# sikoba/babble

Hardware: AMD Instinct MI355X
Metric: ECDSA event verifies/sec (higher is better)
Workload: dtype u32; 1 GPU; C2: VerifyBatch of 1M signed Events per GPU (64 creators, 1x64-B tx, ~446-B bodies); per-key tables rebuilt every step; events_per_gpu=1000000, creators=64, parallelism=single, batches_in_flight=2

## Files before the change

### babble_amd/csrc/kernels.hip

```cpp
#include <hip/hip_runtime.h>
#include <stdint.h>

#include <algorithm>
#include <cstdlib>

#include "evjson.h"
#include "hostscalar.h"

#include "verify_core.h"


#ifndef BV_SHA_WAVES
#define BV_SHA_WAVES 1
#endif
__global__ void __launch_bounds__(256, BV_SHA_WAVES) k_sha256(uint64_t n_msgs, const uint8_t *__restrict__ bytes,
                                                const uint64_t *__restrict__ off,
                                                uint32_t *__restrict__ digest_words, uint64_t max_len) {
  const uint64_t m = (uint64_t)blockIdx.x * blockDim.x + threadIdx.x;
  if (m < n_msgs && off[m + 1] - off[m] <= max_len) sha256_one(m, bytes, off, digest_words);
}

__global__ void __launch_bounds__(256) k_put_digests(uint64_t n, const uint64_t *__restrict__ idx,
                                                     const uint32_t *__restrict__ vals, uint32_t *__restrict__ dig) {
  const uint64_t t = (uint64_t)blockIdx.x * blockDim.x + threadIdx.x;
// ... 391 lines not shown
__global__ void __launch_bounds__(256) k_table_pair_g(const uint32_t *__restrict__ sub, uint32_t *__restrict__ table,
                                                      uint4 *__restrict__ pscr, uint32_t j, uint32_t c0) {
  constexpr uint32_t E = 16, NS = 1u << L, ENT = 1u << (W - 1);
  const uint32_t c = c0 + blockIdx.x, t = threadIdx.x;
  const uint32_t *s_lo = sub + (uint64_t)(2 * j) * NS * BV_ENTRY_U32;
  const uint32_t *s_hi = s_lo + (uint64_t)NS * BV_ENTRY_U32;
  __shared__ fe sT[511];
  uint4 *ps = pscr + (uint64_t)blockIdx.x * E * 2 * 256 + t;
  fe acc;
  fe_set(acc, 1);
#pragma unroll 1
  for (uint32_t e = 0; e < E; e++) {
    const uint32_t d = k12_digit(4096u * c + 256u * e + t, ENT), lo = d & (NS - 1), hi = d >> L;
    fe x1, y1, x2, y2, H;
    pair_load(s_lo, s_hi, lo, hi, x1, y1, x2, y2);
    pair_denominator(H, pair_kind(lo, hi), x1, x2);
    ps[(2 * e) * 256] = make_uint4(acc.v[0], acc.v[1], acc.v[2], acc.v[3]);
    ps[(2 * e + 1) * 256] = make_uint4(acc.v[4], acc.v[5], acc.v[6], acc.v[7]);
    fe_mul(acc, acc, H);
  }
  fe q = acc;
  block_inverse<256>(sT, q, t);
  uint32_t *base = table + (uint64_t)j * ENT * BV_ENTRY_U32;
#pragma unroll 1
  for (int e = (int)E - 1; e >= 0; e--) {
    const uint32_t d = k12_digit(4096u * c + 256u * e + t, ENT), lo = d & (NS - 1), hi = d >> L;
    const int kind = pair_kind(lo, hi);
    fe x1, y1, x2, y2, H, Hinv, pre;
    pair_load(s_lo, s_hi, lo, hi, x1, y1, x2, y2);
    pair_denominator(H, kind, x1, x2);
    const uint4 p0 = ps[(2 * e) * 256], p1 = ps[(2 * e + 1) * 256];
    pre.v[0] = p0.x; pre.v[1] = p0.y; pre.v[2] = p0.z; pre.v[3] = p0.w;
    pre.v[4] = p1.x; pre.v[5] = p1.y; pre.v[6] = p1.z; pre.v[7] = p1.w;
    fe_mul(Hinv, q, pre);
    fe_mul(q, q, H);
    pair_store(base + (uint64_t)d * BV_ENTRY_U32, nullptr, kind, x1, y1, x2, y2, Hinv);
  }
}

__global__ void __launch_bounds__(256) k_sinv(uint64_t n_items, uint32_t M, const uint32_t *__restrict__ s_be,
                                              const uint8_t *__restrict__ pre, uint32_t *__restrict__ w_out) {
  const uint64_t T = (uint64_t)gridDim.x * blockDim.x;
  const uint64_t t = (uint64_t)blockIdx.x * blockDim.x + threadIdx.x;
  sinv_thread(t, T, n_items, M, s_be, pre, w_out);
}

__device__ __forceinline__ void write_status(uint64_t i, uint64_t hi, uint8_t st, uint8_t *status, uint64_t *bits) {
  if (i < hi) status[i] = st;
  const uint64_t mask = __ballot(i < hi && st == BV_ACCEPT);
  if ((threadIdx.x & 63) == 0 && i < hi) bits[i >> 6] = mask;
}

#ifndef BV_GWAVES
#define BV_GWAVES 1
#endif
#ifndef BV_LWAVES
#define BV_LWAVES 1
#endif
__global__ void __launch_bounds__(256) k_glv_split(uint64_t n_items, const uint32_t *__restrict__ r_be,
                                                   const uint32_t *__restrict__ w_in, uint32_t *__restrict__ u12) {
  const uint64_t i = (uint64_t)blockIdx.x * blockDim.x + threadIdx.x;
  if (i < n_items) glv_split_item(i, r_be, w_in, u12);
}

template <bool LAT, bool SPLIT>
__global__ void __launch_bounds__(256, LAT ? BV_LWAVES : BV_GWAVES) k_verify_g(uint64_t n_items, uint64_t lo, uint64_t hi,
                                                  const uint32_t *__restrict__ item_key,
                                                  const uint32_t *__restrict__ r_be, const uint32_t *__restrict__ s_be,
                                                  const uint8_t *__restrict__ pre, const uint8_t *__restrict__ kstatus,
                                                  const uint32_t *__restrict__ item_msg,
                                                  const uint32_t *__restrict__ digest_words,
                                                  const uint32_t *__restrict__ w_in, uint32_t *__restrict__ u12,
                                                  const uint32_t *__restrict__ g_table, uint32_t *__restrict__ rg) {
  const uint64_t i = lo + (uint64_t)blockIdx.x * blockDim.x + threadIdx.x;
  if (i < hi)
    verify_item_g<LAT, SPLIT>(i, n_items, item_key, r_be, s_be, pre, kstatus, item_msg, digest_words, w_in, u12,
                              g_table, rg);
}

#ifndef BV_QWAVES
#define BV_QWAVES 4
#endif
template <int W, int NWIN, bool LAT>
__global__ void __launch_bounds__(256, LAT ? BV_LWAVES : BV_QWAVES) k_verify_q(uint64_t n_items, uint64_t lo, uint64_t hi,
                                                  const uint32_t *__restrict__ item_key,
                                                  const uint32_t *__restrict__ r_be, const uint32_t *__restrict__ s_be,
                                                  const uint8_t *__restrict__ pre, const uint8_t *__restrict__ kstatus,
                                                  const uint32_t *__restrict__ u12,
                                                  const uint32_t *__restrict__ key_table,
                                                  const uint64_t *__restrict__ key_tabs,
                                                  const uint32_t *__restrict__ rg, uint8_t *__restrict__ status,
                                                  uint64_t *__restrict__ bits) {
  const uint64_t i = lo + (uint64_t)blockIdx.x * blockDim.x + threadIdx.x;
  uint8_t st = BV_REJECT;
  if (i < hi)
    st = verify_item_q<W, NWIN, LAT>(i, n_items, item_key, r_be, s_be, pre, kstatus, u12, key_table, key_tabs, rg);
  write_status(i, hi, st, status, bits);
}

template <int W, int NWIN, bool LAT>
__global__ void __launch_bounds__(256, LAT ? BV_LWAVES : BV_QWAVES) k_verify_qf(uint64_t n_items, uint64_t lo, uint64_t hi,
                                                   const uint32_t *__restrict__ item_key,
                                                   const uint32_t *__restrict__ r_be, const uint32_t *__restrict__ s_be,
                                                   const uint8_t *__restrict__ pre, const uint8_t *__restrict__ kstatus,
                                                   const uint32_t *__restrict__ w_in,
                                                   const uint32_t *__restrict__ key_table,
                                                   const uint64_t *__restrict__ key_tabs, uint32_t *__restrict__ rq) {
// ... 960 lines not shown
```

### babble_amd/csrc/point.h

```cpp
#pragma once
#include "field.h"

struct gej {
  fe X, Y, Z;
};

DEV void gej_double(gej &r, const gej &a) {
  fe A, B, C, D, E, F, t;
  fe_sqr(A, a.X);
  fe_sqr(B, a.Y);
  fe_sqr(C, B);
  fe_add(t, a.X, B);
  fe_sqr(t, t);
  fe_sub(t, t, A);
  fe_sub(t, t, C);
  fe_dbl(D, t);
  fe_dbl(E, A);
  fe_add(E, E, A);
  fe_sqr(F, E);
  fe Z3;
  fe_mul(Z3, a.Y, a.Z);
  fe_dbl(r.Z, Z3);
  fe_dbl(t, D);
  fe_sub(r.X, F, t);
// ... 149 lines not shown
  }
  fe_dbl(I, H);
  fe_sqr(I, I);
  fe_mul(J, H, I);
  fe_dbl(rr, rr);
  fe_mul(V, U1, I);
  fe_add(t, r.Z, b.Z);
  fe_sqr(t, t);
  fe_sub(t, t, Z1Z1);
  fe_sub(t, t, Z2Z2);
  fe_mul(r.Z, t, H);
  fe_sqr(t, rr);
  fe_sub(t, t, J);
  fe_sub(t, t, V);
  fe_sub(r.X, t, V);
  fe_sub(t, V, r.X);
  fe_mul(t, rr, t);
  fe_mul(J, S1, J);
  fe_dbl(J, J);
  fe_sub(r.Y, t, J);
}

struct gexz {
  fe X, Y, ZZ, ZZZ;
};

DEV void gexz_double(gexz &r, const gexz &a) {
  fe U, V, W, S, M, t;
  fe_dbl(U, a.Y);
  fe_sqr(V, U);
  fe_mul(W, U, V);
  fe_mul(S, a.X, V);
  fe_sqr(M, a.X);
  fe_dbl(t, M);
  fe_add(M, M, t);
  fe_sqr(t, M);
  fe_dbl(r.X, S);
  fe_sub(r.X, t, r.X);
  fe_sub(t, S, r.X);
  fe_mul(t, M, t);
  fe_mul(U, W, a.Y);
  fe_sub(r.Y, t, U);
  fe_mul(r.ZZ, V, a.ZZ);
  fe_mul(r.ZZZ, W, a.ZZZ);
}

DEV void gexz_set_ge(gexz &r, const fe &x, const fe &y) {
  r.X = x;
  r.Y = y;
  fe_set(r.ZZ, 1);
  fe_set(r.ZZZ, 1);
}

DEV void gexz_add_ge(gexz &r, bool &inf, const fe &x2, const fe &y2, bool xz_only = false) {
  if (inf) {
    gexz_set_ge(r, x2, y2);
    inf = false;
    return;
  }
  fe P, R, PP, PPP, Q, t;
  fe_mul(P, x2, r.ZZ);
  fe_sub(P, P, r.X);
  fe_mul(R, y2, r.ZZZ);
  fe_sub(R, R, r.Y);
  if (fe_is_zero(P)) {
    if (fe_is_zero(R)) {
      gexz d;
      gexz_double(d, r);
      r = d;
    } else {
      inf = true;
    }
    return;
  }
  fe_sqr(PP, P);
  fe_mul(PPP, P, PP);
  fe_mul(Q, r.X, PP);
  fe_mul(r.ZZ, r.ZZ, PP);
  fe_sqr(t, R);
  fe_sub(t, t, PPP);
  fe_sub(t, t, Q);
  fe_sub(r.X, t, Q);
  if (xz_only) return;
  fe_sub(t, Q, r.X);
  fe_mul(t, R, t);
  fe_mul(r.ZZZ, r.ZZZ, PPP);
  fe_mul(PPP, r.Y, PPP);
  fe_sub(r.Y, t, PPP);
}

DEV void gexz_add_ge_lat(gexz &r, bool &inf, const fe &x2, const fe &y2) {
#if defined(__HIP_DEVICE_COMPILE__)
  if (inf) {
    gexz_set_ge(r, x2, y2);
    inf = false;
    return;
  }
  fe P, R, PP, RR, PPP, Q, ZZ3, t, u;
  fe_mul_mul_zip_asm(P, x2, r.ZZ, R, y2, r.ZZZ);
  fe_sub(P, P, r.X);
  fe_sub(R, R, r.Y);
  if (fe_is_zero(P)) {
    if (fe_is_zero(R)) {
      gexz d;
      gexz_double(d, r);
      r = d;
    } else {
      inf = true;
    }
    return;
  }
  fe_sqr_sqr_zip_asm(PP, P, RR, R);
  fe_mul_mul_mul_zip_asm(PPP, P, PP, Q, r.X, PP, ZZ3, r.ZZ, PP);
  r.ZZ = ZZ3;
  fe_sub(t, RR, PPP);
  fe_sub(t, t, Q);
  fe_sub(r.X, t, Q);
  fe_sub(t, Q, r.X);
  fe_mul_mul_mul_zip_asm(t, R, t, u, r.Y, PPP, ZZ3, r.ZZZ, PPP);
  r.ZZZ = ZZ3;
  fe_sub(r.Y, t, u);
#else
  gexz_add_ge(r, inf, x2, y2);
#endif
}

DEV void gexz_add(gexz &r, bool &rinf, const gexz &b, bool binf) {
  if (binf) return;
  if (rinf) {
    r = b;
    rinf = false;
    return;
  }
  fe U1, U2, S1, S2, P, R, PP, PPP, Q, t;
  fe_mul(U1, r.X, b.ZZ);
  fe_mul(U2, b.X, r.ZZ);
  fe_mul(S1, r.Y, b.ZZZ);
  fe_mul(S2, b.Y, r.ZZZ);
  fe_sub(P, U2, U1);
  fe_sub(R, S2, S1);
  if (fe_is_zero(P)) {
// ... 54 lines not shown
  fe_sub(t, Q, r.X);
  fe_mul_mul_mul_zip_asm(t, R, t, u, S1, PPP, r.ZZZ, W12, PPP);
  fe_sub(r.Y, t, u);
#else
  gexz_add(r, rinf, b, binf);
#endif
}

DEV void gexz_sum_ge_lat(gexz &r, bool &rinf, const fe &x1, const fe &y1, bool i1, const fe &x2, const fe &y2,
                         bool i2) {
  rinf = i1 && i2;
  if (i1 || i2) {
    if (!rinf) gexz_set_ge(r, i1 ? x2 : x1, i1 ? y2 : y1);
    return;
  }
  fe P, R;
  fe_sub(P, x2, x1);
  fe_sub(R, y2, y1);
  if (fe_is_zero(P)) {
    if (fe_is_zero(R)) {
      gexz a;
      gexz_set_ge(a, x1, y1);
      gexz_double(r, a);
    } else {
      rinf = true;
    }
    return;
  }
#if defined(__HIP_DEVICE_COMPILE__)
  fe PP, RR, PPP, Q, t, u;
  fe_sqr_sqr_zip_asm(PP, P, RR, R);
  fe_mul_mul_zip_asm(PPP, P, PP, Q, x1, PP);
  fe_sub(t, RR, PPP);
  fe_sub(t, t, Q);
  fe_sub(r.X, t, Q);
  fe_sub(t, Q, r.X);
  fe_mul_mul_zip_asm(t, R, t, u, y1, PPP);
  fe_sub(r.Y, t, u);
  r.ZZ = PP;
  r.ZZZ = PPP;
#else
  gexz_set_ge(r, x1, y1);
  gexz_add_ge(r, rinf, x2, y2);
#endif
}

DEV void gexz_from_gej(gexz &r, const gej &a) {
  r.X = a.X;
  r.Y = a.Y;
  fe_sqr(r.ZZ, a.Z);
  fe_mul(r.ZZZ, r.ZZ, a.Z);
}

template <bool LAT>
DEV void pt_add_ge(gexz &r, bool &inf, const fe &x2, const fe &y2, bool xz_only = false) {
  if (LAT) gexz_add_ge_lat(r, inf, x2, y2);
  else gexz_add_ge(r, inf, x2, y2, xz_only);
}

template <bool LAT>
DEV void gexz_add_ge_aff(gexz &r, bool &inf, const fe &x2, const fe &y2) {
  fe P, R, PP, RR, PPP, Q, t, u, v;
  fe_sub(P, x2, r.X);
  fe_sub(R, y2, r.Y);
  if (fe_is_zero(P)) {
    if (fe_is_zero(R)) {
      gexz d;
      gexz_double(d, r);
      r = d;
    } else {
      inf = true;
    }
    return;
  }
#if defined(__HIP_DEVICE_COMPILE__)
  if (LAT) {
    fe_sqr_sqr_zip_asm(PP, P, RR, R);
    fe_mul_mul_zip_asm(PPP, P, PP, Q, r.X, PP);
  } else
#endif
  {
    fe_sqr(PP, P);
    fe_sqr(RR, R);
    fe_mul(PPP, P, PP);
    fe_mul(Q, r.X, PP);
  }
  fe_sub(t, RR, PPP);
  fe_sub(t, t, Q);
  fe_sub(t, t, Q);
  fe_sub(u, Q, t);
  r.X = t;
  r.ZZ = PP;
  r.ZZZ = PPP;
#if defined(__HIP_DEVICE_COMPILE__)
  if (LAT) {
    fe_mul_mul_zip_asm(t, R, u, v, r.Y, PPP);
  } else
#endif
  {
    fe_mul(t, R, u);
    fe_mul(v, r.Y, PPP);
  }
  fe_sub(r.Y, t, v);
}

template <bool LAT>
DEV void pt_add_ge_step(gexz &r, bool &inf, const fe &x2, const fe &y2, bool take, bool xz_only = false) {
  if (take) pt_add_ge<LAT>(r, inf, x2, y2, xz_only);
}
template <bool LAT>
DEV void pt_add_ge_step(gej &r, bool &inf, const fe &x2, const fe &y2, bool take, bool xz_only = false) {
  if (take) gej_add_ge_sel<LAT>(r, inf, x2, y2);
}
template <bool LAT>
DEV void pt_add_ge(gej &r, bool &inf, const fe &x2, const fe &y2) {
  gej_add_ge_sel<LAT>(r, inf, x2, y2);
}
```

### babble_amd/csrc/verify_core.h

```cpp
#pragma once
#include <type_traits>
#include <stdint.h>

#include "../../include/babbleverify.h"
#include "geometry.h"
#include "coop.h"
#include "point.h"
#include "sha256.h"

#define KS_OK 0
#define KS_EMPTY 1
#define KS_BAD 2

static constexpr uint32_t P_MINUS_N[8] = {0x2FC9BAEEu, 0x402DA172u, 0x50B75FC4u, 0x45512319u,
                                          0x00000001u, 0u, 0u, 0u};

DEV void fe_load_be(fe &r, const uint8_t *b) {
#pragma unroll
  for (int i = 0; i < 8; i++) {
    const uint8_t *q = b + 4 * (7 - i);
    r.v[i] = ((uint32_t)q[0] << 24) | ((uint32_t)q[1] << 16) | ((uint32_t)q[2] << 8) | q[3];
  }
}
DEV void fe_load_be_words(fe &r, const uint32_t *w) {
// ... 505 lines not shown
};

struct lane_park {
#if defined(__HIP_DEVICE_COMPILE__)
  DEV uint4 *slot() {
    __shared__ uint4 park[BV_STAGE_LANES];
    return park + threadIdx.x;
  }
  DEV void put(const uint32_t v[4]) { *slot() = make_uint4(v[0], v[1], v[2], v[3]); }
  DEV void get(uint32_t v[4]) {
    const uint4 a = *slot();
    v[0] = a.x; v[1] = a.y; v[2] = a.z; v[3] = a.w;
  }
#else
  uint32_t buf[4];
  DEV void put(const uint32_t v[4]) {
    for (int c = 0; c < 4; c++) buf[c] = v[c];
  }
  DEV void get(uint32_t v[4]) {
    for (int c = 0; c < 4; c++) v[c] = buf[c];
  }
#endif
};

template <bool PARK>
DEV void glv_half(uint32_t kk[4], int h, const uint32_t k1[4], const uint32_t k2[4], lane_park &park) {
  if (PARK) {
    if (h) park.get(kk);
    else
#pragma unroll
      for (int c = 0; c < 4; c++) kk[c] = k1[c];
  } else {
#pragma unroll
    for (int c = 0; c < 4; c++) kk[c] = h ? k2[c] : k1[c];
  }
}

template <int W, int NL, bool SIGNED>
DEV uint32_t next_digit(uint32_t *u, uint32_t &carry, bool &dneg) {
  constexpr uint32_t ENT = 1u << (W - 1);
  uint32_t d = (u[0] & ((1u << W) - 1u)) + carry;
#pragma unroll
  for (int c = 0; c < NL - 1; c++) u[c] = (u[c] >> W) | (u[c + 1] << (32 - W));
  u[NL - 1] >>= W;
  dneg = false;
  if (SIGNED) {
    carry = d > ENT ? 1u : 0u;
    dneg = carry != 0;
    if (dneg) d = (1u << W) - d;
  }
  return d;
}

template <int W, int NWIN, bool LAT = false, class PT = gej, bool FROM_INF = false, bool FINAL = false>
DEV void g_table_add(PT &R, bool &inf, const uint32_t *tab, uint32_t u[8]) {
  constexpr uint32_t ENT = 1u << (W - 1);
  static_assert(W * NWIN >= 257 && W < 32, "signed G windows must absorb the last carry");
  uint32_t carry = 0;
  if constexpr ((BV_LOOKUP_PIPE & 1) && !LAT && std::is_same<PT, gexz>::value) {
    entry_stage stage;
    bool dneg;
    uint32_t d = next_digit<W, 8, true>(u, carry, dneg);
    stage.request(tab + (uint64_t)d * BV_ENTRY_U32);
#pragma unroll 1
    for (int j = 0; j < NWIN; j++) {
      fe x, y;
      stage.take(x, y);
      const uint32_t dj = d;
      const bool nj = dneg;
      if (j + 1 < NWIN) {
        d = next_digit<W, 8, true>(u, carry, dneg);
        stage.request(tab + ((uint64_t)(j + 1) * ENT + d) * BV_ENTRY_U32);
      }
      fe_cneg_canon(y, nj);
      if constexpr (FROM_INF) {
        if (j == 1 && !inf) {
          if (dj != 0) gexz_add_ge_aff<LAT>(R, inf, x, y);
          continue;
        }
      }
      pt_add_ge_step<LAT>(R, inf, x, y, dj != 0, FINAL && j == NWIN - 1);
    }
    return;
  }
  for (int j = 0; j < NWIN; j++) {
    uint32_t d = (u[0] & ((1u << W) - 1u)) + carry;
#pragma unroll
    for (int c = 0; c < 7; c++) u[c] = (u[c] >> W) | (u[c + 1] << (32 - W));
    u[7] >>= W;
    carry = d > ENT ? 1u : 0u;
    const bool dneg = carry != 0;
    if (dneg) d = (1u << W) - d;
    const uint32_t *e = tab + ((uint64_t)j * ENT + d) * BV_ENTRY_U32;
    fe x, y;
    fe_load4(x, e);
    fe_load4(y, e + 8);
    fe_cneg_canon(y, dneg);
    if constexpr (FROM_INF) {
      if (j == 1 && !inf) {
        if (d != 0) gexz_add_ge_aff<LAT>(R, inf, x, y);
        continue;
      }
    }
    pt_add_ge_step<LAT>(R, inf, x, y, d != 0, FINAL && j == NWIN - 1);
  }
}

DEV void load_k(uint32_t k1[4], uint32_t k2[4], uint32_t &signs, const uint32_t *u12, uint64_t i) {
  const uint4 *q = (const uint4 *)(u12 + (uint64_t)BV_U_STRIDE * i);
  uint4 a = q[0], b = q[1], c = q[2];
  k1[0] = a.x; k1[1] = a.y; k1[2] = a.z; k1[3] = a.w;
  k2[0] = b.x; k2[1] = b.y; k2[2] = b.z; k2[3] = b.w;
  signs = c.x;
}

#define RG_WORDS 33
DEV void rg_store(uint32_t *rg, uint64_t n, uint64_t i, const gexz &R, bool inf) {
#pragma unroll
  for (int k = 0; k < 8; k++) {
    rg[(uint64_t)k * n + i] = R.X.v[k];
    rg[(uint64_t)(8 + k) * n + i] = R.Y.v[k];
    rg[(uint64_t)(16 + k) * n + i] = R.ZZ.v[k];
    rg[(uint64_t)(24 + k) * n + i] = R.ZZZ.v[k];
  }
  rg[(uint64_t)32 * n + i] = inf ? 1u : 0u;
}
DEV void rg_load(const uint32_t *rg, uint64_t n, uint64_t i, gexz &R, bool &inf) {
#pragma unroll
  for (int k = 0; k < 8; k++) {
    R.X.v[k] = rg[(uint64_t)k * n + i];
    R.Y.v[k] = rg[(uint64_t)(8 + k) * n + i];
    R.ZZ.v[k] = rg[(uint64_t)(16 + k) * n + i];
    R.ZZZ.v[k] = rg[(uint64_t)(24 + k) * n + i];
  }
  inf = rg[(uint64_t)32 * n + i] != 0;
}

DEV void glv_split_item(uint64_t i, const uint32_t *r_be, const uint32_t *w_in, uint32_t *u12) {
  sc w, r, b;
  const uint4 *q = (const uint4 *)(w_in + 8 * i);
  const uint4 x = q[0], y = q[1];
  w.v[0] = x.x; w.v[1] = x.y; w.v[2] = x.z; w.v[3] = x.w;
  w.v[4] = y.x; w.v[5] = y.y; w.v[6] = y.z; w.v[7] = y.w;
  sc_load_be_words(r, r_be + 8 * i);
  sc_mont(b, r, w);
  uint32_t k1[4], k2[4], signs;
  glv_split(k1, k2, signs, b);
  uint4 *o = (uint4 *)(u12 + (uint64_t)BV_U_STRIDE * i);
  o[0] = make_uint4(k1[0], k1[1], k1[2], k1[3]);
  o[1] = make_uint4(k2[0], k2[1], k2[2], k2[3]);
  o[2] = make_uint4(signs, 0u, 0u, 0u);
}

template <bool LAT = false, bool SPLIT = false>
DEV void verify_item_g(uint64_t i, uint64_t n, const uint32_t *item_key, const uint32_t *r_be, const uint32_t *s_be,
                       const uint8_t *pre, const uint8_t *kstatus, const uint32_t *item_msg,
                       const uint32_t *digest_words, const uint32_t *w_in, uint32_t *u12, const uint32_t *g_table,
                       uint32_t *rg) {
  fe r;
  if (classify_item(i, item_key, r_be, s_be, pre, kstatus, r) != 0xFF) return;
  uint32_t u[8];
  if (SPLIT) {
    sc w, e, a;
    const uint4 *q = (const uint4 *)(w_in + 8 * i);
    const uint4 x = q[0], y = q[1];
    w.v[0] = x.x; w.v[1] = x.y; w.v[2] = x.z; w.v[3] = x.w;
    w.v[4] = y.x; w.v[5] = y.y; w.v[6] = y.z; w.v[7] = y.w;
    sc_load_be_words(e, digest_words + 8 * (uint64_t)item_msg[i]);
    sc_mont(a, e, w);
#pragma unroll
    for (int k = 0; k < 8; k++) u[k] = a.v[k];
  } else {
    uint32_t k1[4], k2[4], signs;
    item_scalars(i, r_be, item_msg, digest_words, w_in, u, k1, k2, signs);
    uint4 *q = (uint4 *)(u12 + (uint64_t)BV_U_STRIDE * i);
    q[0] = make_uint4(k1[0], k1[1], k1[2], k1[3]);
    q[1] = make_uint4(k2[0], k2[1], k2[2], k2[3]);
    q[2] = make_uint4(signs, 0u, 0u, 0u);
  }
  gexz R;
  bool inf = true;
  fe_set(R.X, 0);
  fe_set(R.Y, 0);
  fe_set(R.ZZ, 0);
  fe_set(R.ZZZ, 0);
  g_table_add<BV_GW, BV_GNWIN, LAT, gexz, true>(R, inf, g_table, u);
  rg_store(rg, n, i, R, inf);
}

template <int W, int NWIN, bool SIGNED, bool LAT = false, class PT = gexz>
DEV void key_table_add(PT &R, bool &inf, const uint32_t *tab, uint32_t k[4], bool neg, bool phi = false,
                       bool from_inf = false, bool last = false) {
  constexpr uint32_t ENT = SIGNED ? (1u << (W - 1)) : (1u << W);
  static_assert(!SIGNED || W * NWIN >= 129, "signed windows must absorb the last carry");
  uint32_t carry = 0;
  if constexpr ((BV_LOOKUP_PIPE & 2) && !LAT && std::is_same<PT, gexz>::value) {
    entry_stage stage;
    bool dneg;
    uint32_t d = next_digit<W, 4, SIGNED>(k, carry, dneg);
    stage.request(tab + (uint64_t)d * BV_ENTRY_U32);
#pragma unroll 1
    for (int j = 0; j < NWIN; j++) {
      fe x, y;
      stage.take(x, y);
      const uint32_t dj = d;
      const bool nj = dneg != neg;
      if (j + 1 < NWIN) {
        d = next_digit<W, 4, SIGNED>(k, carry, dneg);
        stage.request(tab + ((uint64_t)(j + 1) * ENT + d) * BV_ENTRY_U32);
      }
      if (phi) {
        fe beta;
        fe_load(beta, FE_BETA);
        fe_mul(x, x, beta);
      }
      fe_cneg_canon(y, nj);
      if (from_inf && j == 1 && !inf) {
        if (dj != 0) gexz_add_ge_aff<LAT>(R, inf, x, y);
        continue;
      }
      pt_add_ge_step<LAT>(R, inf, x, y, dj != 0, last && j == NWIN - 1);
    }
    return;
  }
  constexpr bool fold = !LAT;
  if (!fold && neg) fe_neg(R.Y, R.Y);
  for (int j = 0; j < NWIN; j++) {
    uint32_t d = (k[0] & ((1u << W) - 1u)) + carry;
    k[0] = (k[0] >> W) | (k[1] << (32 - W));
    k[1] = (k[1] >> W) | (k[2] << (32 - W));
    k[2] = (k[2] >> W) | (k[3] << (32 - W));
    k[3] >>= W;
    bool dneg = false;
    if (SIGNED) {
      carry = d > ENT ? 1u : 0u;
      if (carry) {
        d = (1u << W) - d;
        dneg = true;
      }
    }
    const uint32_t *e = tab + ((uint64_t)j * ENT + d) * BV_ENTRY_U32;
    fe x, y;
    fe_load4(x, e);
    fe_load4(y, e + 8);
    if (phi) {
      fe beta;
      fe_load(beta, FE_BETA);
      fe_mul(x, x, beta);
    }
    fe_cneg_canon(y, dneg != (fold && neg));
    if constexpr (std::is_same<PT, gexz>::value) {
      if (from_inf && j == 1 && !inf) {
        if (d != 0) gexz_add_ge_aff<LAT>(R, inf, x, y);
        continue;
      }
    }
    pt_add_ge_step<LAT>(R, inf, x, y, d != 0, last && j == NWIN - 1);
  }
  if (!fold && neg) fe_neg(R.Y, R.Y);
}

template <int W, int NWIN, bool LAT = false>
DEV uint8_t verify_item_q(uint64_t i, uint64_t n, const uint32_t *item_key, const uint32_t *r_be,
                          const uint32_t *s_be, const uint8_t *pre, const uint8_t *kstatus, const uint32_t *u12,
                          const uint32_t *key_table, const uint64_t *key_tabs, const uint32_t *rg) {
  constexpr bool SIGNED = W != BV_KW;
  constexpr bool KC = W == BV_KCW;
  constexpr uint64_t half =
      SIGNED ? ((uint64_t)NWIN * (1ull << (W - 1)) + 1) * BV_ENTRY_U32 : (uint64_t)NWIN * (1ull << W) * BV_ENTRY_U32;
  static_assert(W != BV_K12W || half == BV_K12HALF_U32, "K12 geometry");
  static_assert(!KC || half == BV_KCHALF_U32, "KC geometry");
  fe r;
  const uint8_t st = classify_item(i, item_key, r_be, s_be, pre, kstatus, r);
  if (st != 0xFF) return st;
  uint32_t k1[4], k2[4], signs;
  load_k(k1, k2, signs, u12, i);
  gexz R;
  bool inf;
  rg_load(rg, n, i, R, inf);
  const uint32_t *tab = key_tabs ? (const uint32_t *)key_tabs[item_key[i]]
                                 : key_table + (uint64_t)item_key[i] * (KC ? 1 : 2) * half;
  if (!tab) return BV_DEFERRED;
  constexpr bool PARK = (BV_LOOKUP_PIPE & 2) && !LAT;
  lane_park park;
  if (PARK) park.put(k2);
#pragma unroll 1
  for (int h = 0; h < 2; h++) {
    uint32_t kk[4];
    glv_half<PARK>(kk, h, k1, k2, park);
    key_table_add<W, NWIN, SIGNED, LAT>(R, inf, tab + (h && !KC ? half : 0), kk, (signs >> h) & 1u, KC && h, false,
                                        h == 1);
  }
  fe_load_be_words(r, r_be + 8 * i);
  return final_check(R, inf, r) ? BV_ACCEPT : BV_REJECT;
}

template <int W, int NWIN, bool LAT = false>
DEV void verify_item_qfirst(uint64_t i, uint64_t n, const uint32_t *item_key, const uint32_t *r_be,
                            const uint32_t *s_be, const uint8_t *pre, const uint8_t *kstatus, const uint32_t *w_in,
                            const uint32_t *key_table, const uint64_t *key_tabs, uint32_t *rq) {
  constexpr bool SIGNED = W != BV_KW;
  constexpr bool KC = W == BV_KCW;
  constexpr uint64_t half =
      SIGNED ? ((uint64_t)NWIN * (1ull << (W - 1)) + 1) * BV_ENTRY_U32 : (uint64_t)NWIN * (1ull << W) * BV_ENTRY_U32;
  fe r;
  if (classify_item(i, item_key, r_be, s_be, pre, kstatus, r) != 0xFF) return;
  uint32_t k1[4], k2[4], signs;
  {
    sc w, rs, b;
    const uint4 *q = (const uint4 *)(w_in + 8 * i);
    const uint4 x = q[0], y = q[1];
    w.v[0] = x.x; w.v[1] = x.y; w.v[2] = x.z; w.v[3] = x.w;
    w.v[4] = y.x; w.v[5] = y.y; w.v[6] = y.z; w.v[7] = y.w;
    sc_load_be_words(rs, r_be + 8 * i);
    sc_mont(b, rs, w);
    glv_split(k1, k2, signs, b);
  }
  gexz R;
  bool inf = true;
  fe_set(R.X, 0);
  fe_set(R.Y, 0);
  fe_set(R.ZZ, 0);
  fe_set(R.ZZZ, 0);
  const uint32_t *tab = key_tabs ? (const uint32_t *)key_tabs[item_key[i]]
                                 : key_table + (uint64_t)item_key[i] * (KC ? 1 : 2) * half;
  if (!tab) {
    rq[(uint64_t)32 * n + i] = 2u;
    return;
  }
  constexpr bool PARK = (BV_LOOKUP_PIPE & 2) && !LAT;
  lane_park park;
  if (PARK) park.put(k2);
#pragma unroll 1
  for (int h = 0; h < 2; h++) {
    uint32_t kk[4];
    glv_half<PARK>(kk, h, k1, k2, park);
    key_table_add<W, NWIN, SIGNED, LAT>(R, inf, tab + (h && !KC ? half : 0), kk, (signs >> h) & 1u, KC && h,
                                        h == 0);
  }
  rg_store(rq, n, i, R, inf);
}

template <bool LAT = false>
DEV uint8_t verify_item_gfinish(uint64_t i, uint64_t n, const uint32_t *item_key, const uint32_t *r_be,
                                const uint32_t *s_be, const uint8_t *pre, const uint8_t *kstatus,
                                const uint32_t *item_msg, const uint32_t *digest_words, const uint32_t *w_in,
                                const uint32_t *g_table, const uint32_t *rq) {
  fe r;
  const uint8_t st = classify_item(i, item_key, r_be, s_be, pre, kstatus, r);
  if (st != 0xFF) return st;
  if (rq[(uint64_t)32 * n + i] == 2u) return BV_DEFERRED;
  uint32_t u[8];
  {
    sc w, e, a;
    const uint4 *q = (const uint4 *)(w_in + 8 * i);
    const uint4 x = q[0], y = q[1];
    w.v[0] = x.x; w.v[1] = x.y; w.v[2] = x.z; w.v[3] = x.w;
    w.v[4] = y.x; w.v[5] = y.y; w.v[6] = y.z; w.v[7] = y.w;
    sc_load_be_words(e, digest_words + 8 * (uint64_t)item_msg[i]);
    sc_mont(a, e, w);
#pragma unroll
    for (int k = 0; k < 8; k++) u[k] = a.v[k];
  }
  gexz R;
  bool inf;
  rg_load(rq, n, i, R, inf);
  g_table_add<BV_GW, BV_GNWIN, LAT, gexz, false, true>(R, inf, g_table, u);
  fe_load_be_words(r, r_be + 8 * i);
  return final_check(R, inf, r) ? BV_ACCEPT : BV_REJECT;
}

template <bool LAT = false>
DEV uint8_t verify_item_gq_kc(uint64_t i, const uint32_t *item_key, const uint32_t *r_be, const uint32_t *s_be,
                              const uint8_t *pre, const uint8_t *kstatus, const uint32_t *item_msg,
                              const uint32_t *digest_words, const uint32_t *w_in, const uint32_t *g_table,
                              const uint64_t *key_tabs) {
  fe r;
  const uint8_t st = classify_item(i, item_key, r_be, s_be, pre, kstatus, r);
  if (st != 0xFF) return st;
  const uint32_t *tab = (const uint32_t *)key_tabs[item_key[i]];
  if (!tab) return BV_DEFERRED;
  uint32_t u[8], k1[4], k2[4], signs;
  item_scalars(i, r_be, item_msg, digest_words, w_in, u, k1, k2, signs);
  gexz R;
  bool inf = true;
  fe_set(R.X, 0);
  fe_set(R.Y, 0);
  fe_set(R.ZZ, 0);
  fe_set(R.ZZZ, 0);
  g_table_add<BV_GW, BV_GNWIN, LAT, gexz, true>(R, inf, g_table, u);
  constexpr bool PARK = (BV_LOOKUP_PIPE & 2) && !LAT;
  lane_park park;
  if (PARK) park.put(k2);
#pragma unroll 1
  for (int h = 0; h < 2; h++) {
    uint32_t kk[4];
    glv_half<PARK>(kk, h, k1, k2, park);
    key_table_add<BV_KCW, BV_KCNWIN, true, LAT>(R, inf, tab, kk, (signs >> h) & 1u, h != 0, false, h == 1);
  }
  fe_load_be_words(r, r_be + 8 * i);
  return final_check(R, inf, r) ? BV_ACCEPT : BV_REJECT;
}

template <bool LAT = false>
DEV uint8_t verify_item_generic(uint64_t i, const uint32_t *item_key, const uint32_t *r_be, const uint32_t *s_be,
                                const uint8_t *pre, const uint8_t *kstatus, const uint32_t *kxy,
                                const uint32_t *item_msg, const uint32_t *digest_words, const uint32_t *w_in,
                                const uint32_t *g_table) {
  fe r;
  const uint8_t st = classify_item(i, item_key, r_be, s_be, pre, kstatus, r);
  if (st != 0xFF) return st;
  const uint32_t k = item_key[i];
  uint32_t u1[8], k1[4], k2[4], signs;
  item_scalars(i, r_be, item_msg, digest_words, w_in, u1, k1, k2, signs);
  fe q1x, q1y, q2x, q2y, beta;
  fe_load(q1x, kxy + 16 * k);
  fe_load(q1y, kxy + 16 * k + 8);
  fe_load(beta, FE_BETA);
  fe_mul(q2x, q1x, beta);
  q2y = q1y;
  if (signs & 1u) fe_neg(q1y, q1y);
  if (signs & 2u) fe_neg(q2y, q2y);
  gej R;
  bool inf = true;
  fe_set(R.X, 0);
  fe_set(R.Y, 0);
  fe_set(R.Z, 0);
  for (int bit = 127; bit >= 0; bit--) {
    if (!inf) gej_double_sel<LAT>(R, R);
    if ((k1[bit >> 5] >> (bit & 31)) & 1u) gej_add_ge_sel<LAT>(R, inf, q1x, q1y);
    if ((k2[bit >> 5] >> (bit & 31)) & 1u) gej_add_ge_sel<LAT>(R, inf, q2x, q2y);
  }
  g_table_add<BV_GW, BV_GNWIN, LAT>(R, inf, g_table, u1);
  return final_check(R, inf, r) ? BV_ACCEPT : BV_REJECT;
}

DEV void sinv_one(sc &w, const sc &s) {
  sc t, one;
#pragma unroll
  for (int k = 0; k < 8; k++) one.v[k] = k == 0 ? 1u : 0u;
  sc_inverse_var(t, s);
  sc_mont(w, t, one);
}

DEV void scalars_from(const sc &w, const sc &e, const sc &r, uint32_t u1[8], uint32_t k1[4], uint32_t k2[4],
                      uint32_t &signs) {
  sc a, b;
  sc_mont(a, e, w);
  sc_mont(b, r, w);
#pragma unroll
  for (int k = 0; k < 8; k++) u1[k] = a.v[k];
// ... 99 lines not shown
```

Baseline: 536.2 million verifies/s.

## Defer point-add exception checks to a cold recompute path on ZZ==0

```diff
diff --git a/babble_amd/csrc/kernels.hip b/babble_amd/csrc/kernels.hip
--- a/babble_amd/csrc/kernels.hip
+++ b/babble_amd/csrc/kernels.hip
@@ -467,7 +467,7 @@
 }
 
 #ifndef BV_GWAVES
-#define BV_GWAVES 1
+#define BV_GWAVES (BV_LAZY_EXC ? 4 : 1)
 #endif
 #ifndef BV_LWAVES
 #define BV_LWAVES 1
diff --git a/babble_amd/csrc/point.h b/babble_amd/csrc/point.h
--- a/babble_amd/csrc/point.h
+++ b/babble_amd/csrc/point.h
@@ -225,7 +225,12 @@
   fe_set(r.ZZZ, 1);
 }
 
-DEV void gexz_add_ge(gexz &r, bool &inf, const fe &x2, const fe &y2, bool xz_only = false) {
+#ifndef BV_LAZY_EXC
+#define BV_LAZY_EXC 1
+#endif
+
+template <bool CHECK>
+DEV void gexz_add_ge_t(gexz &r, bool &inf, const fe &x2, const fe &y2, bool xz_only) {
   if (inf) {
     gexz_set_ge(r, x2, y2);
     inf = false;
@@ -236,7 +241,7 @@
   fe_sub(P, P, r.X);
   fe_mul(R, y2, r.ZZZ);
   fe_sub(R, R, r.Y);
-  if (fe_is_zero(P)) {
+  if (CHECK && fe_is_zero(P)) {
     if (fe_is_zero(R)) {
       gexz d;
       gexz_double(d, r);
@@ -260,6 +265,9 @@
   fe_mul(r.ZZZ, r.ZZZ, PPP);
   fe_mul(PPP, r.Y, PPP);
   fe_sub(r.Y, t, PPP);
+}
+DEV void gexz_add_ge(gexz &r, bool &inf, const fe &x2, const fe &y2, bool xz_only = false) {
+  gexz_add_ge_t<true>(r, inf, x2, y2, xz_only);
 }
 
 DEV void gexz_add_ge_lat(gexz &r, bool &inf, const fe &x2, const fe &y2) {
@@ -420,18 +428,19 @@
   fe_mul(r.ZZZ, r.ZZ, a.Z);
 }
 
-template <bool LAT>
+template <bool LAT, bool CHECK = true>
 DEV void pt_add_ge(gexz &r, bool &inf, const fe &x2, const fe &y2, bool xz_only = false) {
+  static_assert(CHECK || !LAT, "the unchecked step is a throughput form");
   if (LAT) gexz_add_ge_lat(r, inf, x2, y2);
-  else gexz_add_ge(r, inf, x2, y2, xz_only);
-}
-
-template <bool LAT>
+  else gexz_add_ge_t<CHECK>(r, inf, x2, y2, xz_only);
+}
+
+template <bool LAT, bool CHECK = true>
 DEV void gexz_add_ge_aff(gexz &r, bool &inf, const fe &x2, const fe &y2) {
   fe P, R, PP, RR, PPP, Q, t, u, v;
   fe_sub(P, x2, r.X);
   fe_sub(R, y2, r.Y);
-  if (fe_is_zero(P)) {
+  if (CHECK && fe_is_zero(P)) {
     if (fe_is_zero(R)) {
       gexz d;
       gexz_double(d, r);
@@ -472,12 +481,13 @@
   fe_sub(r.Y, t, v);
 }
 
-template <bool LAT>
+template <bool LAT, bool CHECK = true>
 DEV void pt_add_ge_step(gexz &r, bool &inf, const fe &x2, const fe &y2, bool take, bool xz_only = false) {
-  if (take) pt_add_ge<LAT>(r, inf, x2, y2, xz_only);
-}
-template <bool LAT>
+  if (take) pt_add_ge<LAT, CHECK>(r, inf, x2, y2, xz_only);
+}
+template <bool LAT, bool CHECK = true>
 DEV void pt_add_ge_step(gej &r, bool &inf, const fe &x2, const fe &y2, bool take, bool xz_only = false) {
+  static_assert(CHECK, "the unchecked step is XYZZ only");
   if (take) gej_add_ge_sel<LAT>(r, inf, x2, y2);
 }
 template <bool LAT>
diff --git a/babble_amd/csrc/verify_core.h b/babble_amd/csrc/verify_core.h
--- a/babble_amd/csrc/verify_core.h
+++ b/babble_amd/csrc/verify_core.h
@@ -581,7 +581,8 @@
   return d;
 }
 
-template <int W, int NWIN, bool LAT = false, class PT = gej, bool FROM_INF = false, bool FINAL = false>
+template <int W, int NWIN, bool LAT = false, class PT = gej, bool FROM_INF = false, bool FINAL = false,
+          bool CHECK = true>
 DEV void g_table_add(PT &R, bool &inf, const uint32_t *tab, uint32_t u[8]) {
   constexpr uint32_t ENT = 1u << (W - 1);
   static_assert(W * NWIN >= 257 && W < 32, "signed G windows must absorb the last carry");
@@ -604,11 +605,11 @@
       fe_cneg_canon(y, nj);
       if constexpr (FROM_INF) {
         if (j == 1 && !inf) {
-          if (dj != 0) gexz_add_ge_aff<LAT>(R, inf, x, y);
+          if (dj != 0) gexz_add_ge_aff<LAT, CHECK>(R, inf, x, y);
           continue;
         }
       }
-      pt_add_ge_step<LAT>(R, inf, x, y, dj != 0, FINAL && j == NWIN - 1);
+      pt_add_ge_step<LAT, CHECK>(R, inf, x, y, dj != 0, FINAL && j == NWIN - 1);
     }
     return;
   }
@@ -627,11 +628,11 @@
     fe_cneg_canon(y, dneg);
     if constexpr (FROM_INF) {
       if (j == 1 && !inf) {
-        if (d != 0) gexz_add_ge_aff<LAT>(R, inf, x, y);
+        if (d != 0) gexz_add_ge_aff<LAT, CHECK>(R, inf, x, y);
         continue;
       }
     }
-    pt_add_ge_step<LAT>(R, inf, x, y, d != 0, FINAL && j == NWIN - 1);
+    pt_add_ge_step<LAT, CHECK>(R, inf, x, y, d != 0, FINAL && j == NWIN - 1);
   }
 }
 
@@ -681,13 +682,23 @@
   o[2] = make_uint4(signs, 0u, 0u, 0u);
 }
 
-template <bool LAT = false, bool SPLIT = false>
-DEV void verify_item_g(uint64_t i, uint64_t n, const uint32_t *item_key, const uint32_t *r_be, const uint32_t *s_be,
-                       const uint8_t *pre, const uint8_t *kstatus, const uint32_t *item_msg,
-                       const uint32_t *digest_words, const uint32_t *w_in, uint32_t *u12, const uint32_t *g_table,
-                       uint32_t *rg) {
-  fe r;
-  if (classify_item(i, item_key, r_be, s_be, pre, kstatus, r) != 0xFF) return;
+#if defined(BV_COUNT_REDO) && !defined(__HIP_DEVICE_COMPILE__)
+static uint64_t bv_redo_count = 0;
+#endif
+DEV bool chain_hit_exception(const gexz &R, bool inf) {
+  const bool hit = !inf && fe_is_zero(R.ZZ);
+#if defined(BV_COUNT_REDO) && !defined(__HIP_DEVICE_COMPILE__)
+  if (hit) bv_redo_count++;
+#endif
+  return hit;
+}
+template <bool LAT>
+DEV constexpr bool lazy_exc() { return BV_LAZY_EXC != 0 && !LAT; }
+#define BV_COLD __host__ __device__ __attribute__((noinline)) inline
+
+template <bool LAT, bool SPLIT, bool CHECK>
+DEV void item_g_sum(gexz &R, bool &inf, uint64_t i, const uint32_t *r_be, const uint32_t *item_msg,
+                    const uint32_t *digest_words, const uint32_t *w_in, uint32_t *u12, const uint32_t *g_table) {
   uint32_t u[8];
   if (SPLIT) {
     sc w, e, a;
@@ -707,17 +718,44 @@
     q[1] = make_uint4(k2[0], k2[1], k2[2], k2[3]);
     q[2] = make_uint4(signs, 0u, 0u, 0u);
   }
-  gexz R;
-  bool inf = true;
+  inf = true;
   fe_set(R.X, 0);
   fe_set(R.Y, 0);
   fe_set(R.ZZ, 0);
   fe_set(R.ZZZ, 0);
-  g_table_add<BV_GW, BV_GNWIN, LAT, gexz, true>(R, inf, g_table, u);
+  g_table_add<BV_GW, BV_GNWIN, LAT, gexz, true, false, CHECK>(R, inf, g_table, u);
+}
+
+template <bool SPLIT>
+BV_COLD void item_g_checked(uint64_t i, uint64_t n, const uint32_t *r_be, const uint32_t *item_msg,
+                            const uint32_t *digest_words, const uint32_t *w_in, uint32_t *u12,
+                            const uint32_t *g_table, uint32_t *rg) {
+  gexz R;
+  bool inf;
+  item_g_sum<false, SPLIT, true>(R, inf, i, r_be, item_msg, digest_words, w_in, u12, g_table);
   rg_store(rg, n, i, R, inf);
 }
 
-template <int W, int NWIN, bool SIGNED, bool LAT = false, class PT = gexz>
+template <bool LAT = false, bool SPLIT = false>
+DEV void verify_item_g(uint64_t i, uint64_t n, const uint32_t *item_key, const uint32_t *r_be, const uint32_t *s_be,
+                       const uint8_t *pre, const uint8_t *kstatus, const uint32_t *item_msg,
+                       const uint32_t *digest_words, const uint32_t *w_in, uint32_t *u12, const uint32_t *g_table,
+                       uint32_t *rg) {
+  fe r;
+  if (classify_item(i, item_key, r_be, s_be, pre, kstatus, r) != 0xFF) return;
+  gexz R;
+  bool inf;
+  item_g_sum<LAT, SPLIT, !lazy_exc<LAT>()>(R, inf, i, r_be, item_msg, digest_words, w_in, u12, g_table);
+  if constexpr (lazy_exc<LAT>()) {
+    if (chain_hit_exception(R, inf)) {
+      item_g_checked<SPLIT>(i, n, r_be, item_msg, digest_words, w_in, u12, g_table, rg);
+      return;
+    }
+  }
+  rg_store(rg, n, i, R, inf);
+}
+
+template <int W, int NWIN, bool SIGNED, bool LAT = false, class PT = gexz, bool CHECK = true>
 DEV void key_table_add(PT &R, bool &inf, const uint32_t *tab, uint32_t k[4], bool neg, bool phi = false,
                        bool from_inf = false, bool last = false) {
   constexpr uint32_t ENT = SIGNED ? (1u << (W - 1)) : (1u << W);
@@ -745,10 +783,10 @@
       }
       fe_cneg_canon(y, nj);
       if (from_inf && j == 1 && !inf) {
-        if (dj != 0) gexz_add_ge_aff<LAT>(R, inf, x, y);
+        if (dj != 0) gexz_add_ge_aff<LAT, CHECK>(R, inf, x, y);
         continue;
       }
-      pt_add_ge_step<LAT>(R, inf, x, y, dj != 0, last && j == NWIN - 1);
+      pt_add_ge_step<LAT, CHECK>(R, inf, x, y, dj != 0, last && j == NWIN - 1);
     }
     return;
   }
@@ -780,13 +818,46 @@
     fe_cneg_canon(y, dneg != (fold && neg));
     if constexpr (std::is_same<PT, gexz>::value) {
       if (from_inf && j == 1 && !inf) {
-        if (d != 0) gexz_add_ge_aff<LAT>(R, inf, x, y);
+        if (d != 0) gexz_add_ge_aff<LAT, CHECK>(R, inf, x, y);
         continue;
       }
     }
-    pt_add_ge_step<LAT>(R, inf, x, y, d != 0, last && j == NWIN - 1);
+    pt_add_ge_step<LAT, CHECK>(R, inf, x, y, d != 0, last && j == NWIN - 1);
   }
   if (!fold && neg) fe_neg(R.Y, R.Y);
+}
+
+template <int W, int NWIN, bool LAT, bool CHECK>
+DEV void item_q_sum(gexz &R, bool &inf, uint64_t i, uint64_t n, const uint32_t *u12, const uint32_t *rg,
+                    const uint32_t *tab) {
+  constexpr bool SIGNED = W != BV_KW;
+  constexpr bool KC = W == BV_KCW;
+  constexpr uint64_t half =
+      SIGNED ? ((uint64_t)NWIN * (1ull << (W - 1)) + 1) * BV_ENTRY_U32 : (uint64_t)NWIN * (1ull << W) * BV_ENTRY_U32;
+  uint32_t k1[4], k2[4], signs;
+  load_k(k1, k2, signs, u12, i);
+  rg_load(rg, n, i, R, inf);
+  constexpr bool PARK = (BV_LOOKUP_PIPE & 2) && !LAT;
+  lane_park park;
+  if (PARK) park.put(k2);
+#pragma unroll 1
+  for (int h = 0; h < 2; h++) {
+    uint32_t kk[4];
+    glv_half<PARK>(kk, h, k1, k2, park);
+    key_table_add<W, NWIN, SIGNED, LAT, gexz, CHECK>(R, inf, tab + (h && !KC ? half : 0), kk, (signs >> h) & 1u,
+                                                     KC && h, false, h == 1);
+  }
+}
+
+template <int W, int NWIN>
+BV_COLD uint8_t item_q_checked(uint64_t i, uint64_t n, const uint32_t *r_be, const uint32_t *u12, const uint32_t *rg,
+                               const uint32_t *tab) {
+  gexz R;
+  bool inf;
+  item_q_sum<W, NWIN, false, true>(R, inf, i, n, u12, rg, tab);
+  fe r;
+  fe_load_be_words(r, r_be + 8 * i);
+  return final_check(R, inf, r) ? BV_ACCEPT : BV_REJECT;
 }
 
 template <int W, int NWIN, bool LAT = false>
@@ -802,14 +873,42 @@
   fe r;
   const uint8_t st = classify_item(i, item_key, r_be, s_be, pre, kstatus, r);
   if (st != 0xFF) return st;
-  uint32_t k1[4], k2[4], signs;
-  load_k(k1, k2, signs, u12, i);
-  gexz R;
-  bool inf;
-  rg_load(rg, n, i, R, inf);
   const uint32_t *tab = key_tabs ? (const uint32_t *)key_tabs[item_key[i]]
                                  : key_table + (uint64_t)item_key[i] * (KC ? 1 : 2) * half;
   if (!tab) return BV_DEFERRED;
+  gexz R;
+  bool inf;
+  item_q_sum<W, NWIN, LAT, !lazy_exc<LAT>()>(R, inf, i, n, u12, rg, tab);
+  if constexpr (lazy_exc<LAT>()) {
+    if (chain_hit_exception(R, inf)) return item_q_checked<W, NWIN>(i, n, r_be, u12, rg, tab);
+  }
+  fe_load_be_words(r, r_be + 8 * i);
+  return final_check(R, inf, r) ? BV_ACCEPT : BV_REJECT;
+}
+
+template <int W, int NWIN, bool LAT, bool CHECK>
+DEV void item_qfirst_sum(gexz &R, bool &inf, uint64_t i, const uint32_t *r_be, const uint32_t *w_in,
+                         const uint32_t *tab) {
+  constexpr bool SIGNED = W != BV_KW;
+  constexpr bool KC = W == BV_KCW;
+  constexpr uint64_t half =
+      SIGNED ? ((uint64_t)NWIN * (1ull << (W - 1)) + 1) * BV_ENTRY_U32 : (uint64_t)NWIN * (1ull << W) * BV_ENTRY_U32;
+  uint32_t k1[4], k2[4], signs;
+  {
+    sc w, rs, b;
+    const uint4 *q = (const uint4 *)(w_in + 8 * i);
+    const uint4 x = q[0], y = q[1];
+    w.v[0] = x.x; w.v[1] = x.y; w.v[2] = x.z; w.v[3] = x.w;
+    w.v[4] = y.x; w.v[5] = y.y; w.v[6] = y.z; w.v[7] = y.w;
+    sc_load_be_words(rs, r_be + 8 * i);
+    sc_mont(b, rs, w);
+    glv_split(k1, k2, signs, b);
+  }
+  inf = true;
+  fe_set(R.X, 0);
+  fe_set(R.Y, 0);
+  fe_set(R.ZZ, 0);
+  fe_set(R.ZZZ, 0);
   constexpr bool PARK = (BV_LOOKUP_PIPE & 2) && !LAT;
   lane_park park;
   if (PARK) park.put(k2);
@@ -817,11 +916,18 @@
   for (int h = 0; h < 2; h++) {
     uint32_t kk[4];
     glv_half<PARK>(kk, h, k1, k2, park);
-    key_table_add<W, NWIN, SIGNED, LAT>(R, inf, tab + (h && !KC ? half : 0), kk, (signs >> h) & 1u, KC && h, false,
-                                        h == 1);
-  }
-  fe_load_be_words(r, r_be + 8 * i);
-  return final_check(R, inf, r) ? BV_ACCEPT : BV_REJECT;
+    key_table_add<W, NWIN, SIGNED, LAT, gexz, CHECK>(R, inf, tab + (h && !KC ? half : 0), kk, (signs >> h) & 1u,
+                                                     KC && h, h == 0);
+  }
+}
+
+template <int W, int NWIN>
+BV_COLD void item_qfirst_checked(uint64_t i, uint64_t n, const uint32_t *r_be, const uint32_t *w_in,
+                                 const uint32_t *tab, uint32_t *rq) {
+  gexz R;
+  bool inf;
+  item_qfirst_sum<W, NWIN, false, true>(R, inf, i, r_be, w_in, tab);
+  rg_store(rq, n, i, R, inf);
 }
 
 template <int W, int NWIN, bool LAT = false>
@@ -834,40 +940,53 @@
       SIGNED ? ((uint64_t)NWIN * (1ull << (W - 1)) + 1) * BV_ENTRY_U32 : (uint64_t)NWIN * (1ull << W) * BV_ENTRY_U32;
   fe r;
   if (classify_item(i, item_key, r_be, s_be, pre, kstatus, r) != 0xFF) return;
-  uint32_t k1[4], k2[4], signs;
-  {
-    sc w, rs, b;
-    const uint4 *q = (const uint4 *)(w_in + 8 * i);
-    const uint4 x = q[0], y = q[1];
-    w.v[0] = x.x; w.v[1] = x.y; w.v[2] = x.z; w.v[3] = x.w;
-    w.v[4] = y.x; w.v[5] = y.y; w.v[6] = y.z; w.v[7] = y.w;
-    sc_load_be_words(rs, r_be + 8 * i);
-    sc_mont(b, rs, w);
-    glv_split(k1, k2, signs, b);
-  }
-  gexz R;
-  bool inf = true;
-  fe_set(R.X, 0);
-  fe_set(R.Y, 0);
-  fe_set(R.ZZ, 0);
-  fe_set(R.ZZZ, 0);
   const uint32_t *tab = key_tabs ? (const uint32_t *)key_tabs[item_key[i]]
                                  : key_table + (uint64_t)item_key[i] * (KC ? 1 : 2) * half;
   if (!tab) {
     rq[(uint64_t)32 * n + i] = 2u;
     return;
   }
-  constexpr bool PARK = (BV_LOOKUP_PIPE & 2) && !LAT;
-  lane_park park;
-  if (PARK) park.put(k2);
-#pragma unroll 1
-  for (int h = 0; h < 2; h++) {
-    uint32_t kk[4];
-    glv_half<PARK>(kk, h, k1, k2, park);
-    key_table_add<W, NWIN, SIGNED, LAT>(R, inf, tab + (h && !KC ? half : 0), kk, (signs >> h) & 1u, KC && h,
-                                        h == 0);
+  gexz R;
+  bool inf;
+  item_qfirst_sum<W, NWIN, LAT, !lazy_exc<LAT>()>(R, inf, i, r_be, w_in, tab);
+  if constexpr (lazy_exc<LAT>()) {
+    if (chain_hit_exception(R, inf)) {
+      item_qfirst_checked<W, NWIN>(i, n, r_be, w_in, tab, rq);
+      return;
+    }
   }
   rg_store(rq, n, i, R, inf);
+}
+
+template <bool LAT, bool CHECK>
+DEV void item_gfinish_sum(gexz &R, bool &inf, uint64_t i, uint64_t n, const uint32_t *item_msg,
+                          const uint32_t *digest_words, const uint32_t *w_in, const uint32_t *g_table,
+                          const uint32_t *rq) {
+  uint32_t u[8];
+  {
+    sc w, e, a;
+    const uint4 *q = (const uint4 *)(w_in + 8 * i);
+    const uint4 x = q[0], y = q[1];
+    w.v[0] = x.x; w.v[1] = x.y; w.v[2] = x.z; w.v[3] = x.w;
+    w.v[4] = y.x; w.v[5] = y.y; w.v[6] = y.z; w.v[7] = y.w;
+    sc_load_be_words(e, digest_words + 8 * (uint64_t)item_msg[i]);
+    sc_mont(a, e, w);
+#pragma unroll
+    for (int k = 0; k < 8; k++) u[k] = a.v[k];
+  }
+  rg_load(rq, n, i, R, inf);
+  g_table_add<BV_GW, BV_GNWIN, LAT, gexz, false, true, CHECK>(R, inf, g_table, u);
+}
+
+BV_COLD uint8_t item_gfinish_checked(uint64_t i, uint64_t n, const uint32_t *r_be, const uint32_t *item_msg,
+                                     const uint32_t *digest_words, const uint32_t *w_in, const uint32_t *g_table,
+                                     const uint32_t *rq) {
+  gexz R;
+  bool inf;
+  item_gfinish_sum<false, true>(R, inf, i, n, item_msg, digest_words, w_in, g_table, rq);
+  fe r;
+  fe_load_be_words(r, r_be + 8 * i);
+  return final_check(R, inf, r) ? BV_ACCEPT : BV_REJECT;
 }
 
 template <bool LAT = false>
@@ -879,22 +998,48 @@
   const uint8_t st = classify_item(i, item_key, r_be, s_be, pre, kstatus, r);
   if (st != 0xFF) return st;
   if (rq[(uint64_t)32 * n + i] == 2u) return BV_DEFERRED;
-  uint32_t u[8];
-  {
-    sc w, e, a;
-    const uint4 *q = (const uint4 *)(w_in + 8 * i);
-    const uint4 x = q[0], y = q[1];
-    w.v[0] = x.x; w.v[1] = x.y; w.v[2] = x.z; w.v[3] = x.w;
-    w.v[4] = y.x; w.v[5] = y.y; w.v[6] = y.z; w.v[7] = y.w;
-    sc_load_be_words(e, digest_words + 8 * (uint64_t)item_msg[i]);
-    sc_mont(a, e, w);
-#pragma unroll
-    for (int k = 0; k < 8; k++) u[k] = a.v[k];
-  }
   gexz R;
   bool inf;
-  rg_load(rq, n, i, R, inf);
-  g_table_add<BV_GW, BV_GNWIN, LAT, gexz, false, true>(R, inf, g_table, u);
+  item_gfinish_sum<LAT, !lazy_exc<LAT>()>(R, inf, i, n, item_msg, digest_words, w_in, g_table, rq);
+  if constexpr (lazy_exc<LAT>()) {
+    if (chain_hit_exception(R, inf))
+      return item_gfinish_checked(i, n, r_be, item_msg, digest_words, w_in, g_table, rq);
+  }
+  fe_load_be_words(r, r_be + 8 * i);
+  return final_check(R, inf, r) ? BV_ACCEPT : BV_REJECT;
+}
+
+template <bool LAT, bool CHECK>
+DEV void item_gq_kc_sum(gexz &R, bool &inf, uint64_t i, const uint32_t *r_be, const uint32_t *item_msg,
+                        const uint32_t *digest_words, const uint32_t *w_in, const uint32_t *g_table,
+                        const uint32_t *tab) {
+  uint32_t u[8], k1[4], k2[4], signs;
+  item_scalars(i, r_be, item_msg, digest_words, w_in, u, k1, k2, signs);
+  inf = true;
+  fe_set(R.X, 0);
+  fe_set(R.Y, 0);
+  fe_set(R.ZZ, 0);
+  fe_set(R.ZZZ, 0);
+  g_table_add<BV_GW, BV_GNWIN, LAT, gexz, true, false, CHECK>(R, inf, g_table, u);
+  constexpr bool PARK = (BV_LOOKUP_PIPE & 2) && !LAT;
+  lane_park park;
+  if (PARK) park.put(k2);
+#pragma unroll 1
+  for (int h = 0; h < 2; h++) {
+    uint32_t kk[4];
+    glv_half<PARK>(kk, h, k1, k2, park);
+    key_table_add<BV_KCW, BV_KCNWIN, true, LAT, gexz, CHECK>(R, inf, tab, kk, (signs >> h) & 1u, h != 0, false,
+                                                             h == 1);
+  }
+}
+
+BV_COLD uint8_t item_gq_kc_checked(uint64_t i, const uint32_t *r_be, const uint32_t *item_msg,
+                                   const uint32_t *digest_words, const uint32_t *w_in, const uint32_t *g_table,
+                                   const uint32_t *tab) {
+  gexz R;
+  bool inf;
+  item_gq_kc_sum<false, true>(R, inf, i, r_be, item_msg, digest_words, w_in, g_table, tab);
+  fe r;
   fe_load_be_words(r, r_be + 8 * i);
   return final_check(R, inf, r) ? BV_ACCEPT : BV_REJECT;
 }
@@ -909,23 +1054,12 @@
   if (st != 0xFF) return st;
   const uint32_t *tab = (const uint32_t *)key_tabs[item_key[i]];
   if (!tab) return BV_DEFERRED;
-  uint32_t u[8], k1[4], k2[4], signs;
-  item_scalars(i, r_be, item_msg, digest_words, w_in, u, k1, k2, signs);
   gexz R;
-  bool inf = true;
-  fe_set(R.X, 0);
-  fe_set(R.Y, 0);
-  fe_set(R.ZZ, 0);
-  fe_set(R.ZZZ, 0);
-  g_table_add<BV_GW, BV_GNWIN, LAT, gexz, true>(R, inf, g_table, u);
-  constexpr bool PARK = (BV_LOOKUP_PIPE & 2) && !LAT;
-  lane_park park;
-  if (PARK) park.put(k2);
-#pragma unroll 1
-  for (int h = 0; h < 2; h++) {
-    uint32_t kk[4];
-    glv_half<PARK>(kk, h, k1, k2, park);
-    key_table_add<BV_KCW, BV_KCNWIN, true, LAT>(R, inf, tab, kk, (signs >> h) & 1u, h != 0, false, h == 1);
+  bool inf;
+  item_gq_kc_sum<LAT, !lazy_exc<LAT>()>(R, inf, i, r_be, item_msg, digest_words, w_in, g_table, tab);
+  if constexpr (lazy_exc<LAT>()) {
+    if (chain_hit_exception(R, inf))
+      return item_gq_kc_checked(i, r_be, item_msg, digest_words, w_in, g_table, tab);
   }
   fe_load_be_words(r, r_be + 8 * i);
   return final_check(R, inf, r) ? BV_ACCEPT : BV_REJECT;
```

Measured after the change: 540.9 million verifies/s (median of 6 runs). Within noise of the previous version (+0.9%).
